# bharatlytics/faceRecognition_InfrenceEngine

Measured on AMD Instinct MI355X. Metric: faces/sec end-to-end @1080p, higher is better.
Workload: dtype f16

## Files before the change

### facerecognition_infrenceengine_amd/csrc/common.h

```cpp
#pragma once
#include <hip/hip_runtime.h>
#include <atomic>
#include <cstdarg>
#include <cstdint>
#include <cstdio>
#include <type_traits>
#include "../../include/frhip.h"

#define FR_WAVE 64

void fr_set_error(const char* fmt, ...);

#define FR_REQUIRE(cond, ...)                      \
    do {                                           \
        if (!(cond)) {                             \
            fr_set_error(__VA_ARGS__);             \
            return FR_E_INVALID;                   \
        }                                          \
    } while (0)

#define FR_CHECK_LAUNCH(name)                                                     \
    do {                                                                          \
        hipError_t e_ = hipGetLastError();                                        \
        if (e_ != hipSuccess) {                                                   \
// ... 22 lines not shown
typedef _Float16 half2v __attribute__((ext_vector_type(2)));
typedef float float4v __attribute__((ext_vector_type(4)));
typedef float float16v __attribute__((ext_vector_type(16)));
typedef int int2v __attribute__((ext_vector_type(2)));
typedef int int4v __attribute__((ext_vector_type(4)));
typedef int int8v __attribute__((ext_vector_type(8)));
typedef __attribute__((address_space(3))) void* lds_ptr_t;
typedef unsigned long long u64_unaligned __attribute__((aligned(1)));

template <int N, int I = 0, class F>
__device__ __forceinline__ void static_for(F&& f) {
    if constexpr (I < N) {
        f(std::integral_constant<int, I>{});
        static_for<N, I + 1>(f);
    }
}

#define FR_PIN() __builtin_amdgcn_sched_barrier(0)

__device__ __forceinline__ float wave_sum(float v) {
#pragma unroll
    for (int o = 32; o > 0; o >>= 1) v += __shfl_xor(v, o, 64);
    return v;
}

__device__ __forceinline__ __amdgpu_buffer_rsrc_t buffer_rsrc(const void* p, unsigned bytes) {
    return __builtin_amdgcn_make_buffer_rsrc((void*)p, 0, bytes, 0x00020000);
}

__device__ __forceinline__ float4v mfma16(const int4v& a, const int4v& b, float4v c) {
    return __builtin_amdgcn_mfma_f32_16x16x32_f16(__builtin_bit_cast(half8, a), __builtin_bit_cast(half8, b), c, 0, 0, 0);
}

__device__ __forceinline__ int pack_fp8x4(float a, float b, float c, float d) {
    a = __builtin_amdgcn_fmed3f(a, -448.f, 448.f); b = __builtin_amdgcn_fmed3f(b, -448.f, 448.f);
    c = __builtin_amdgcn_fmed3f(c, -448.f, 448.f); d = __builtin_amdgcn_fmed3f(d, -448.f, 448.f);
    int v = 0;
    v = __builtin_amdgcn_cvt_pk_fp8_f32(a, b, v, false);
    v = __builtin_amdgcn_cvt_pk_fp8_f32(c, d, v, true);
    return v;
}

__device__ __forceinline__ bool slot_valid(const int32_t* seg_counts, int seg_len, int q) {
    const int seg = q / seg_len;
    return q - seg * seg_len < seg_counts[seg];
}
```

### facerecognition_infrenceengine_amd/csrc/conv_stage28.hip

```cpp
#include "common.h"
#include <type_traits>

namespace {

constexpr int S28_W = 28, S28_TH = 14, S28_C = 128;
constexpr int S28_HROWS = 16 * 32;
constexpr int S28_PLANE = S28_HROWS * 128;
constexpr int S28_SLOT = 128 * 64;
constexpr int S28_STEPS = 36;
constexpr int S28_PRM = 10 * 128 * 4;
constexpr int S28_RING = 2 * S28_PLANE, S28_PRMO = S28_RING + 3 * S28_SLOT;
constexpr int S28_LDS = S28_PRMO + S28_PRM;
constexpr int S28_PX = S28_TH * S28_W;
constexpr int S28_IMG = 784 * S28_C * 2;

struct Stage28P {
    half_t* x; half_t* mid; const half_t* w; const float* prm;
    int B, nconv;
    unsigned xbytes, wbytes;
};

}

__global__ __launch_bounds__(512, 2) void conv_stage28_kernel(Stage28P p) {
#if defined(__HIP_DEVICE_COMPILE__)
    extern __shared__ __attribute__((aligned(16))) char lds[];
    char* ring = lds + S28_RING;
    const float* lprm = reinterpret_cast<const float*>(lds + S28_PRMO);
    const int tid = threadIdx.x;
    const int wave = __builtin_amdgcn_readfirstlane(tid >> 6);
    const int wn = wave & 1, wp = wave >> 1;
    const int n = blockIdx.x;

    __amdgpu_buffer_rsrc_t wrs = buffer_rsrc(p.w, p.wbytes);
    __amdgpu_buffer_rsrc_t xrs = buffer_rsrc(p.x, p.xbytes);
    __amdgpu_buffer_rsrc_t mrs = buffer_rsrc(p.mid, p.xbytes);
    __amdgpu_buffer_rsrc_t prs = buffer_rsrc(p.prm, (unsigned)p.nconv * S28_PRM);

    unsigned wsrc = 0, wwrap = S28_STEPS * S28_SLOT, wback = 0;
    auto issue_w = [&](int slot, int ln) {
        __builtin_amdgcn_raw_ptr_buffer_load_lds(wrs, (lds_ptr_t)(ring + slot * S28_SLOT + wave * 1024), 16,
                                                 wsrc < p.wbytes ? (unsigned)(wave * 1024 + ln * 16) : 0x80000000u, wsrc, 0, 0);
        wsrc += S28_SLOT;
        if (wsrc == wwrap) wsrc = wback;
    };
    auto halo_lane = [&](int ln) -> unsigned {
        const int lrow = ln >> 3, ch = ln & 7, q = wave & 3;
        const unsigned out = (unsigned)((q == 0) & (lrow == 0)) | (unsigned)((q == 3) & (lrow >= 5));
        return ((unsigned)((lrow - 1) * 256 + ((ch ^ ((lrow + 4 * ((wave >> 2) & 1)) & 7)) << 4)) & (out - 1u)) | (out << 31);
    };
    auto issue_halo = [&](__amdgpu_buffer_rsrc_t rs, int plane, int i, int y0, unsigned lt, bool src_ok) {
        int n_ = n;
        asm volatile("" : "+s"(n_));
        const int hy = 2 * i + (wave >> 2), iy = y0 - 1 + hy;
        const bool ok = src_ok && (unsigned)iy < 28u;
        const unsigned so = (unsigned)(((n_ * 28 + iy) * 28 + (wave & 3) * 8) * 256 + plane * 128);
        __builtin_amdgcn_raw_ptr_buffer_load_lds(rs, (lds_ptr_t)(lds + plane * S28_PLANE + (hy * 4 + (wave & 3)) * 1024), 16,
                                                 ok ? lt + so : 0x80000000u, 0, 0, 16);
    };
    auto issue_prm = [&](int conv, int ln) {
        if (wave < 5)
            __builtin_amdgcn_raw_ptr_buffer_load_lds(prs, (lds_ptr_t)(lds + S28_PRMO + wave * 1024), 16, (unsigned)(wave * 1024 + ln * 16), conv * S28_PRM, 0, 0);
    };

    {
        const int ln = tid & 63;
        issue_w(0, ln);
        issue_w(1, ln);
        issue_w(2, ln);
        issue_prm(0, ln);
        const unsigned lt = halo_lane(ln);
        for (int i = 0; i < 16; ++i) issue_halo(xrs, i >> 3, i & 7, 0, lt, true);
    }

    float4v acc[6][4], accx;
    int4v a0[4], a1[4], bt[3], bx;
    int boff[7];

    auto run = [&](auto role_tag) {
    constexpr int ROLE = decltype(role_tag)::value;
#pragma unroll 1
    for (int pass = 0; pass < 2 * p.nconv; ++pass) {
        const int conv = pass >> 1, hf = pass & 1, y0 = hf * S28_TH;
        int lane = tid & 63;
        asm volatile("" : "+v"(lane));
        const int fr = lane & 15, fq = lane >> 4;
        const bool second = conv & 1;
        __amdgpu_buffer_rsrc_t srs = second ? mrs : xrs;
        __amdgpu_buffer_rsrc_t nxr = hf == 0 ? srs : (second ? xrs : mrs);
        const int nxy0 = hf == 0 ? S28_TH : 0;
        const bool nx_any = hf == 0 || conv + 1 < p.nconv;
        auto nx_ok = [&](int i) { return nx_any && (hf == 0 || !(i == 7 && (wave >> 2) == 1)); };
        half_t* dst = second ? p.x : p.mid;
        const unsigned tile0 = (unsigned)((n * 28 + y0) * 28);
        int a_own = fr * 64 + ((fq ^ (((fr >> 3) & 1) << 1)) << 4);
        asm volatile("" : "+v"(a_own));
        int hb[6];
#pragma unroll
        for (int j = 0; j < 6; ++j) {
            const int px = (wp * 6 + j) * 16 + fr;
            const int oy = px / S28_W, ox = px - oy * S28_W;
            hb[j] = (oy + 1) * 32 + ox + 1;
            asm volatile("" : "+v"(hb[j]));
        }
        auto set_tap_one = [&](int j, int dy, int dx, int plane) {
            int l_ = lane;
            asm volatile("" : "+v"(l_));
            const int h = (j < 6 ? hb[j < 6 ? j : 0] : ((l_ & 15) < 8 ? 14 * 32 + 21 + (l_ & 15) : 33)) + dy * 32 + dx;
            boff[j] = plane * S28_PLANE + h * 128 + (((l_ >> 4) ^ ((((h >> 3) & 4) + h) & 7)) << 4);
        };
        auto rd_a = [&](int slot, int i) {
            return *reinterpret_cast<const int4v*>(ring + slot * S28_SLOT + (wn * 4096 + ((i + wp) & 3) * 1024) + a_own);
        };
        auto rd_b = [&](int gg, int j) { return *reinterpret_cast<const int4v*>(lds + (gg ? (boff[j] ^ 64) : boff[j])); };
        auto co_of = [&](int i) { return wn * 64 + ((i + wp) & 3) * 16 + fq * 4; };

        if (hf == 0) {
            if (pass == 0) asm volatile("s_waitcnt vmcnt(16)" ::: "memory");
            else if (wave >> 2) asm volatile("s_waitcnt vmcnt(2)" ::: "memory");
            else asm volatile("s_waitcnt vmcnt(0)" ::: "memory");
            __builtin_amdgcn_s_barrier();
        }
        auto cls_off = [&](int px) {
            const int oy = px / S28_W, ox = px - oy * S28_W, ho = y0 + oy;
            return ((ho == 0 ? 0 : (ho == 27 ? 2 : 1)) * 3 + (ox == 0 ? 0 : (ox == 27 ? 2 : 1))) * S28_C;
        };
#pragma unroll
        for (int j = 0; j < 6; ++j) {
            const int cj = cls_off((wp * 6 + j) * 16 + fr);
#pragma unroll
            for (int i = 0; i < 4; ++i) acc[j][i] = *reinterpret_cast<const float4v*>(lprm + cj + co_of(i));
        }
        accx = *reinterpret_cast<const float4v*>(lprm + cls_off(fr < 8 ? 384 + fr : 0) + co_of(0));
        auto co8 = [&](int ip) { return wn * 64 + ((ip + (fq & 1) + wp) & 3) * 16 + (fq >> 1) * 8; };
        if (second) {
            int4v r[6][2];
#pragma unroll
            for (int j = 0; j < 6; ++j)
#pragma unroll
                for (int ip = 0; ip < 2; ++ip)
                    r[j][ip] = __builtin_bit_cast(int4v, __builtin_amdgcn_raw_buffer_load_b128(
                        xrs, (tile0 + (unsigned)((wp * 6 + j) * 16 + fr)) * 256u + (unsigned)co8(2 * ip) * 2u, 0, 16));
#pragma unroll
            for (int j = 0; j < 6; ++j)
#pragma unroll
                for (int ip = 0; ip < 2; ++ip) {
                    const auto s0 = __builtin_amdgcn_permlane16_swap((unsigned)r[j][ip][0], (unsigned)r[j][ip][2], false, false);
                    const auto s1 = __builtin_amdgcn_permlane16_swap((unsigned)r[j][ip][1], (unsigned)r[j][ip][3], false, false);
                    const half4 ha = __builtin_bit_cast(half4, int2v{(int)s0[0], (int)s1[0]});
                    const half4 hb_ = __builtin_bit_cast(half4, int2v{(int)s0[1], (int)s1[1]});
#pragma unroll
                    for (int e = 0; e < 4; ++e) { acc[j][2 * ip][e] += (float)ha[e]; acc[j][2 * ip + 1][e] += (float)hb_[e]; }
                }
            const int2v rx = __builtin_bit_cast(int2v, __builtin_amdgcn_raw_buffer_load_b64(
                xrs, fr < 8 ? (tile0 + (unsigned)(384 + fr)) * 256u + (unsigned)co_of(0) * 2u : 0x80000000u, 0, 16));
            const half4 hx = __builtin_bit_cast(half4, rx);
#pragma unroll
            for (int e = 0; e < 4; ++e) accx[e] += (float)hx[e];
        }
        asm volatile("s_waitcnt vmcnt(0)" ::: "memory");
        __builtin_amdgcn_s_barrier();
        wwrap = (unsigned)(conv + 1) * (S28_STEPS * S28_SLOT);
        wback = hf == 0 ? (unsigned)conv * (S28_STEPS * S28_SLOT) : wwrap;

#pragma unroll
        for (int j = 0; j < 7; ++j) set_tap_one(j, -1, -1, 0);
#pragma unroll
        for (int i = 0; i < 4; ++i) a0[i] = rd_a(0, i);
#pragma unroll
        for (int j = 0; j < 3; ++j) bt[j] = rd_b(0, j);
        bx = rd_b(0, 6);

        auto step = [&](int4v (&ac)[4], int4v (&an)[4], int k, int dyn, int dxn, int pln, auto pf_tag) {
            constexpr bool PF = decltype(pf_tag)::value;
            const int gg = k & 1, ngg = (k + 1) & 1, nslot = (k + 1) % 3;
            auto dma = [&]() {
                if constexpr (PF) {
                    if (k < 4) {
                        int l_ = lane;
                        asm volatile("" : "+v"(l_));
                        const unsigned ltp = halo_lane(l_);
                        issue_halo(nxr, 0, 2 * k, nxy0, ltp, nx_ok(2 * k));
                        issue_halo(nxr, 0, 2 * k + 1, nxy0, ltp, nx_ok(2 * k + 1));
                    }
                }
                issue_w(k % 3, lane);
            };
            if constexpr (ROLE == 0) { dma(); FR_PIN(); }
            accx = mfma16(ac[0], bx, accx);
            FR_PIN();
#pragma unroll
            for (int j = 0; j < 6; ++j) {
#pragma unroll
                for (int i = 0; i < 4; ++i) acc[j][i] = mfma16(ac[i], bt[j % 3], acc[j][i]);
                if (j == 0) { an[0] = rd_a(nslot, 0); an[1] = rd_a(nslot, 1); }
                if (j == 1) { an[2] = rd_a(nslot, 2); an[3] = rd_a(nslot, 3); }
                if (j < 3) {
                    bt[j] = rd_b(gg, j + 3);
                } else {
                    if (gg == 1) { set_tap_one(j - 3, dyn, dxn, pln); set_tap_one(j, dyn, dxn, pln); }
                    bt[j - 3] = rd_b(ngg, j - 3);
                    if (j == 5) {
                        if (gg == 1) set_tap_one(6, dyn, dxn, pln);
                        bx = rd_b(ngg, 6);
                    }
                }
                FR_PIN();
                if constexpr (ROLE == 1) { if (j == 3) { dma(); FR_PIN(); } }
            }
        };
        auto row = [&](int it, int plane, auto pf_tag) {
            constexpr bool PF = decltype(pf_tag)::value;
#pragma unroll
            for (int k = 0; k < 6; ++k) {
                if (PF && k >= 1 && k <= 4) asm volatile("s_waitcnt vmcnt(3) lgkmcnt(1)" ::: "memory");
                else asm volatile("s_waitcnt vmcnt(1) lgkmcnt(1)" ::: "memory");
                __builtin_amdgcn_s_barrier();
                FR_PIN();
                const int tt = k >> 1;
                const bool last = tt == 2 && it == 2;
                const int dyn = last ? -1 : (tt < 2 ? it - 1 : it), dxn = tt < 2 ? tt : -1;
                const int pln = last ? (plane ^ 1) & 1 : plane;
                if ((k & 1) == 0) step(a0, a1, k, dyn, dxn, pln, pf_tag);
                else step(a1, a0, k, dyn, dxn, pln, pf_tag);
            }
        };
#pragma unroll 1
        for (int it = 0; it < 3; ++it) row(it, 0, std::false_type{});
        row(0, 1, std::true_type{});
#pragma unroll 1
        for (int it = 1; it < 3; ++it) row(it, 1, std::false_type{});

        asm volatile("s_waitcnt lgkmcnt(0)" ::: "memory");
        __builtin_amdgcn_s_barrier();
        int le = lane;
        asm volatile("" : "+v"(le));
        const unsigned lt = halo_lane(le);
        for (int i = 0; i < 8; ++i) issue_halo(nxr, 1, i, nxy0, lt, nx_ok(i));
        FR_PIN();
        const int fre = le & 15, fqe = le >> 4;
        auto coe = [&](int i) { return wn * 64 + ((i + wp) & 3) * 16 + fqe * 4; };
        float4v sv[4];
#pragma unroll
        for (int i = 0; i < 4; ++i) sv[i] = *reinterpret_cast<const float4v*>(lprm + 9 * S28_C + coe(i));
        auto act = [&](float4v v, int i) {
            if (!second) {
#pragma unroll
                for (int e = 0; e < 4; ++e) v[e] = v[e] > 0.f ? v[e] : v[e] * sv[i][e];
            }
            return __builtin_bit_cast(int2v, half4{(half_t)v[0], (half_t)v[1], (half_t)v[2], (half_t)v[3]});
        };
        auto co8e = [&](int ip) { return wn * 64 + ((ip + (fqe & 1) + wp) & 3) * 16 + (fqe >> 1) * 8; };
#pragma unroll
        for (int j = 0; j < 6; ++j)
#pragma unroll
            for (int ip = 0; ip < 2; ++ip) {
                const int2v pa = act(acc[j][2 * ip], 2 * ip), pb = act(acc[j][2 * ip + 1], 2 * ip + 1);
                const auto s0 = __builtin_amdgcn_permlane16_swap((unsigned)pa[0], (unsigned)pb[0], false, false);
                const auto s1 = __builtin_amdgcn_permlane16_swap((unsigned)pa[1], (unsigned)pb[1], false, false);
                *reinterpret_cast<int4v*>(dst + (size_t)(tile0 + (wp * 6 + j) * 16 + fre) * S28_C + co8e(2 * ip)) =
                    int4v{(int)s0[0], (int)s1[0], (int)s0[1], (int)s1[1]};
            }
        if (fre < 8)
            *reinterpret_cast<int2v*>(dst + (size_t)(tile0 + 384 + fre) * S28_C + coe(0)) = act(accx, 0);
        if (hf == 1) {
            asm volatile("s_waitcnt vmcnt(0)" ::: "memory");
            __builtin_amdgcn_s_barrier();
            if (conv + 1 < p.nconv) {
                issue_prm(conv + 1, lane);
                if (wave >> 2) {
                    issue_halo(nxr, 0, 7, 0, lt, true);
                    issue_halo(nxr, 1, 7, 0, lt, true);
                }
            }
        }
    }
    };
    if ((wp >> 1) == 0) run(std::integral_constant<int, 0>{}); else run(std::integral_constant<int, 1>{});
    asm volatile("s_waitcnt vmcnt(0) lgkmcnt(0)" ::: "memory");
#endif
}

extern "C" size_t fr_conv_stage28_weight_bytes(int nconv) { return nconv > 0 ? (size_t)nconv * S28_STEPS * S28_SLOT : 0; }

__global__ void stage28_pack_weights(const half_t* __restrict__ w, half_t* __restrict__ out) {
    const int e = blockIdx.x * blockDim.x + threadIdx.x;
    if (e >= S28_STEPS * 512) return;
    const int q = e / 512, r = e - q * 512, row = r >> 2, cp = r & 3;
    const int chunk = cp ^ (((row >> 3) & 1) << 1);
    const int plane = q / 18, k = q - plane * 18, tap = k >> 1, gg = k & 1;
    const int4v v = *reinterpret_cast<const int4v*>(w + (size_t)row * 1152 + tap * 128 + plane * 64 + gg * 32 + chunk * 8);
    *reinterpret_cast<int4v*>(out + (size_t)q * 4096 + row * 32 + cp * 8) = v;
}

extern "C" int fr_conv_stage28_pack(const void* w, void* out, fr_stream_t stream) {
    FR_REQUIRE(w && out, "fr_conv_stage28_pack: null pointer");
    stage28_pack_weights<<<fr_cdiv(S28_STEPS * 512, 256), 256, 0, fr_stream(stream)>>>((const half_t*)w, (half_t*)out);
// ... 24 lines not shown
```

### facerecognition_infrenceengine_amd/csrc/conv_walk64.hip

```cpp
#include "common.h"
#include <type_traits>

namespace {

constexpr int K64_RW = 28, K64_RH = 14, K64_C = 64;
constexpr int K64_PX = K64_RW * K64_RH;
constexpr int K64_HALO = 512 * 128;
constexpr int K64_SLOT = 64 * 128;
constexpr int K64_RING = 2 * K64_HALO, K64_PRMO = K64_RING + 3 * K64_SLOT;
constexpr int K64_PRM = 10 * 64 * 4;
constexpr int K64_LDS = K64_PRMO + K64_PRM;

struct Walk64P {
    const half_t* x; const half_t* w; half_t* y;
    const float* bias; const float* slope; const half_t* res;
    int B, HW, Cout, bias_mode;
    int nsplit;
    unsigned xbytes, ybytes, wbytes;
};

}

__global__ __launch_bounds__(512, 2) void conv_walk64_kernel(Walk64P p) {
#if defined(__HIP_DEVICE_COMPILE__)
    extern __shared__ __attribute__((aligned(16))) char lds[];
    char* ring = lds + K64_RING;
    float* lprm = reinterpret_cast<float*>(lds + K64_PRMO);
    const int tid = threadIdx.x;
    const int wave = __builtin_amdgcn_readfirstlane(tid >> 6);
    const int ncg = p.Cout >> 6;
    const int cg = blockIdx.x % ncg, part = (blockIdx.x / ncg) % p.nsplit, n = blockIdx.x / (ncg * p.nsplit);
    const int HW = p.HW, nbx = HW / K64_RW;
    const int reg0 = part * (nbx * (HW / K64_RH) / p.nsplit), nreg = reg0 + nbx * (HW / K64_RH) / p.nsplit;

    __amdgpu_buffer_rsrc_t wrs = buffer_rsrc(p.w, p.wbytes);
    __amdgpu_buffer_rsrc_t xrs = buffer_rsrc(p.x, p.xbytes);

    const unsigned wbase = (unsigned)cg * (9 * K64_SLOT);
    unsigned wq = 0;
    auto issue_w = [&](int slot, int ln) {
        __builtin_amdgcn_raw_ptr_buffer_load_lds(wrs, (lds_ptr_t)(ring + slot * K64_SLOT + wave * 1024), 16,
                                                 (unsigned)(wave * 1024 + ln * 16), wbase + wq * K64_SLOT, 0, 0);
        wq = wq == 8 ? 0 : wq + 1;
    };
    auto halo_lane = [&](int ln, bool left_edge, bool right_edge) -> unsigned {
        const int lrow = ln >> 3, ch = ln & 7, q = wave & 3;
        const unsigned out = (unsigned)((q == 0) & (lrow == 0) & left_edge) | (unsigned)((q == 3) & (lrow == 5) & right_edge) |
                             (unsigned)((q == 3) & (lrow >= 6));
        return ((unsigned)((lrow - 1) * 128 + ((ch ^ ((lrow + 4 * ((wave >> 2) & 1)) & 7)) << 4)) & (out - 1u)) | (out << 31);
    };
    auto issue_halo = [&](int buf, int i, int reg, int ln) {
        int n_ = n;
        asm volatile("" : "+s"(n_));
        const int by = reg / nbx, bx_ = reg - by * nbx;
        const int y0 = by * K64_RH, x0 = bx_ * K64_RW;
        const unsigned lt = halo_lane(ln, x0 == 0, x0 + K64_RW == HW);
        const int hy = 2 * i + (wave >> 2), iy = y0 - 1 + hy;
        const bool ok = reg < nreg && (unsigned)iy < (unsigned)HW;
        const unsigned so = (unsigned)(((n_ * HW + iy) * HW + x0 + (wave & 3) * 8) * 128);
        __builtin_amdgcn_raw_ptr_buffer_load_lds(xrs, (lds_ptr_t)(lds + buf * K64_HALO + (hy * 4 + (wave & 3)) * 1024), 16,
                                                 ok ? lt + so : 0x80000000u, 0, 0, 0);
    };

    {
        const int ln = tid & 63;
        issue_w(0, ln);
        issue_w(1, ln);
        issue_w(2, ln);
        for (int i = 0; i < 8; ++i) issue_halo(reg0 & 1, i, reg0, ln);
        for (int e = tid; e < 640; e += 512) {
            const int r = e >> 6, c = e & 63;
            float v;
            if (r < 9) v = p.bias ? p.bias[(p.bias_mode == 1 ? r * p.Cout : 0) + cg * 64 + c] : 0.f;
            else v = p.slope ? p.slope[cg * 64 + c] : 1.f;
            lprm[e] = v;
        }
    }

    float4v acc[3][4], accx;
    int4v a0[2][4], a1[2][4], b[3][2], bx[2];
    int boff[4];

    auto run = [&](auto role_tag) {
    constexpr int ROLE = decltype(role_tag)::value;
#pragma unroll 1
    for (int reg = reg0; reg < nreg; ++reg) {
        const int cur = reg & 1;
        int lane = tid & 63;
        asm volatile("" : "+v"(lane));
        const int fr = lane & 15, fq = lane >> 4;
        const int by = reg / nbx, bx_ = reg - by * nbx;
        const int y0 = by * K64_RH, x0 = bx_ * K64_RW;
        auto gpix = [&](int px) {
            const int oy = px / K64_RW, ox = px - oy * K64_RW;
            return (unsigned)((n * HW + y0 + oy) * HW + x0 + ox);
        };
        auto cls_off = [&](int px) {
            const int oy = px / K64_RW, ox = px - oy * K64_RW, ho = y0 + oy, wo = x0 + ox;
            return ((ho == 0 ? 0 : (ho == HW - 1 ? 2 : 1)) * 3 + (wo == 0 ? 0 : (wo == HW - 1 ? 2 : 1))) * 64;
        };
        auto ct = [&](int f) { return (f + wave) & 3; };
        auto co8 = [&](int ip) { return ct(2 * ip + (fq & 1)) * 16 + (fq >> 1) * 8; };
        int a_own = fr * 128 + ((fq ^ (fr & 7)) << 4);
        asm volatile("" : "+v"(a_own));
        int hb[3];
#pragma unroll
        for (int t = 0; t < 3; ++t) {
            const int px = (wave * 3 + t) * 16 + fr;
            const int oy = px / K64_RW, ox = px - oy * K64_RW;
            hb[t] = (oy + 1) * 32 + ox + 1;
            asm volatile("" : "+v"(hb[t]));
        }
        auto set_tap_one = [&](int t, int dy, int dx) {
            int l_ = lane;
            asm volatile("" : "+v"(l_));
            const int h = (t < 3 ? hb[t < 3 ? t : 0] : ((l_ & 15) < 8 ? 14 * 32 + 21 + (l_ & 15) : 33)) + dy * 32 + dx;
            boff[t] = cur * K64_HALO + h * 128 + (((l_ >> 4) ^ ((((h >> 3) & 4) + h) & 7)) << 4);
        };
        auto rd_a = [&](int slot, int kh, int i) { return *reinterpret_cast<const int4v*>(ring + slot * K64_SLOT + ct(i) * 2048 + (kh ? (a_own ^ 64) : a_own)); };
        auto rd_b = [&](int kh, int t) { return *reinterpret_cast<const int4v*>(lds + (kh ? (boff[t] ^ 64) : boff[t])); };

        asm volatile("s_waitcnt lgkmcnt(0)" ::: "memory");
        if (reg == reg0) __builtin_amdgcn_s_barrier();
#pragma unroll
        for (int t = 0; t < 3; ++t) {
            const int cj = cls_off((wave * 3 + t) * 16 + fr);
#pragma unroll
            for (int i = 0; i < 4; ++i) acc[t][i] = *reinterpret_cast<const float4v*>(lprm + cj + ct(i) * 16 + fq * 4);
        }
        accx = *reinterpret_cast<const float4v*>(lprm + cls_off(fr < 8 ? 384 + fr : 0) + (wave & 3) * 16 + fq * 4);
        if (p.res) {
            __amdgpu_buffer_rsrc_t rrs = buffer_rsrc(p.res, p.ybytes);
            int4v r[3][2];
#pragma unroll
            for (int t = 0; t < 3; ++t)
#pragma unroll
                for (int ip = 0; ip < 2; ++ip)
                    r[t][ip] = __builtin_bit_cast(int4v, __builtin_amdgcn_raw_buffer_load_b128(
                        rrs, (gpix((wave * 3 + t) * 16 + fr) * (unsigned)p.Cout + (unsigned)(cg * 64 + co8(ip))) * 2u, 0, 16));
            const int2v rx = __builtin_bit_cast(int2v, __builtin_amdgcn_raw_buffer_load_b64(
                rrs, fr < 8 ? (gpix(384 + fr) * (unsigned)p.Cout + (unsigned)(cg * 64 + (wave & 3) * 16 + fq * 4)) * 2u : 0x80000000u, 0, 16));
#pragma unroll
            for (int t = 0; t < 3; ++t)
#pragma unroll
                for (int ip = 0; ip < 2; ++ip) {
                    const auto s0 = __builtin_amdgcn_permlane16_swap((unsigned)r[t][ip][0], (unsigned)r[t][ip][2], false, false);
                    const auto s1 = __builtin_amdgcn_permlane16_swap((unsigned)r[t][ip][1], (unsigned)r[t][ip][3], false, false);
                    const half4 ha = __builtin_bit_cast(half4, int2v{(int)s0[0], (int)s1[0]});
                    const half4 hb_ = __builtin_bit_cast(half4, int2v{(int)s0[1], (int)s1[1]});
#pragma unroll
                    for (int e = 0; e < 4; ++e) { acc[t][2 * ip][e] += (float)ha[e]; acc[t][2 * ip + 1][e] += (float)hb_[e]; }
                }
            const half4 hx = __builtin_bit_cast(half4, rx);
#pragma unroll
            for (int e = 0; e < 4; ++e) accx[e] += (float)hx[e];
        }
        asm volatile("s_waitcnt vmcnt(0)" ::: "memory");
        __builtin_amdgcn_s_barrier();

#pragma unroll
        for (int t = 0; t < 4; ++t) set_tap_one(t, -1, -1);
#pragma unroll
        for (int kh = 0; kh < 2; ++kh) {
#pragma unroll
            for (int i = 0; i < 4; ++i) a0[kh][i] = rd_a(0, kh, i);
#pragma unroll
            for (int t = 0; t < 3; ++t) b[t][kh] = rd_b(kh, t);
            bx[kh] = rd_b(kh, 3);
        }

        auto step = [&](int4v (&ac)[2][4], int4v (&an)[2][4], int s) {
            const int nslot = (s + 1) % 3;
            const int tn = s + 1 < 9 ? s + 1 : 0;
            const int dyn = tn / 3 - 1, dxn = tn % 3 - 1;
            auto dma = [&]() {
                if (s < 8) issue_halo(cur ^ 1, s, reg + 1, lane);
                issue_w(s % 3, lane);
            };
            if constexpr (ROLE == 0) { dma(); FR_PIN(); }
#pragma unroll
            for (int kh = 0; kh < 2; ++kh) {
                accx = mfma16(ac[kh][0], bx[kh], accx);
                FR_PIN();
#pragma unroll
                for (int t = 0; t < 3; ++t) {
#pragma unroll
                    for (int i = 0; i < 4; ++i) acc[t][i] = mfma16(ac[kh][i], b[t][kh], acc[t][i]);
                    if (kh == 0) { an[0][t] = rd_a(nslot, 0, t); if (t == 2) an[0][3] = rd_a(nslot, 0, 3); }
                    else { an[1][t] = rd_a(nslot, 1, t); if (t == 2) an[1][3] = rd_a(nslot, 1, 3); }
                    if (kh == 0) set_tap_one(t, dyn, dxn);
                    b[t][kh] = rd_b(kh, t);
                    if (t == 2) {
                        if (kh == 0) set_tap_one(3, dyn, dxn);
                        bx[kh] = rd_b(kh, 3);
                    }
                    FR_PIN();
                }
                if constexpr (ROLE == 1) { if (kh == 0) { dma(); FR_PIN(); } }
            }
        };
#pragma unroll
        for (int s = 0; s < 9; ++s) {
            asm volatile("s_waitcnt vmcnt(2) lgkmcnt(1)" ::: "memory");
            __builtin_amdgcn_s_barrier();
            FR_PIN();
            if ((s & 1) == 0) step(a0, a1, s); else step(a1, a0, s);
        }

        asm volatile("s_waitcnt lgkmcnt(0)" ::: "memory");
        int le = lane;
        asm volatile("" : "+v"(le));
        const int fre = le & 15, fqe = le >> 4;
        float4v sv[4];
#pragma unroll
        for (int i = 0; i < 4; ++i) sv[i] = *reinterpret_cast<const float4v*>(lprm + 9 * 64 + ct(i) * 16 + fqe * 4);
        auto act = [&](float4v v, const float4v& s_) {
#pragma unroll
            for (int e = 0; e < 4; ++e) v[e] = v[e] > 0.f ? v[e] : v[e] * s_[e];
            return __builtin_bit_cast(int2v, half4{(half_t)v[0], (half_t)v[1], (half_t)v[2], (half_t)v[3]});
        };
        half_t* yo = p.y + cg * 64;
#pragma unroll
        for (int t = 0; t < 3; ++t) {
            const size_t gp = (size_t)gpix((wave * 3 + t) * 16 + fre) * p.Cout;
#pragma unroll
            for (int ip = 0; ip < 2; ++ip) {
                const int2v pa = act(acc[t][2 * ip], sv[2 * ip]), pb = act(acc[t][2 * ip + 1], sv[2 * ip + 1]);
                const auto s0 = __builtin_amdgcn_permlane16_swap((unsigned)pa[0], (unsigned)pb[0], false, false);
                const auto s1 = __builtin_amdgcn_permlane16_swap((unsigned)pa[1], (unsigned)pb[1], false, false);
                *reinterpret_cast<int4v*>(yo + gp + ct(2 * ip + (fqe & 1)) * 16 + (fqe >> 1) * 8) = int4v{(int)s0[0], (int)s1[0], (int)s0[1], (int)s1[1]};
            }
        }
        if (wave < 4 && fre < 8)
            *reinterpret_cast<int2v*>(yo + (size_t)gpix(384 + fre) * p.Cout + wave * 16 + fqe * 4) = act(accx, sv[0]);
    }
    };
    if ((wave >> 2) == 0) run(std::integral_constant<int, 0>{}); else run(std::integral_constant<int, 1>{});
    asm volatile("s_waitcnt vmcnt(0) lgkmcnt(0)" ::: "memory");
#endif
}

extern "C" size_t fr_conv_walk64_weight_bytes(int Cout) { return Cout > 0 ? (size_t)(Cout / 64) * 9 * K64_SLOT : 0; }

__global__ void walk64_pack_weights(const half_t* __restrict__ w, half_t* __restrict__ out, int ncg) {
    const int e = blockIdx.x * blockDim.x + threadIdx.x;
    if (e >= ncg * 9 * 512) return;
    const int q_ = e / 512, r = e - q_ * 512, row = r >> 3, cp = r & 7;
    const int cgi = q_ / 9, tap = q_ - cgi * 9;
    const int chunk = cp ^ (row & 7);
    const int4v v = *reinterpret_cast<const int4v*>(w + (size_t)(cgi * 64 + row) * 576 + tap * 64 + chunk * 8);
    *reinterpret_cast<int4v*>(out + (size_t)q_ * 4096 + row * 64 + cp * 8) = v;
}

extern "C" int fr_conv_walk64_pack(const void* w, void* out, int Cout, fr_stream_t stream) {
    FR_REQUIRE(w && out && Cout > 0 && Cout % 64 == 0, "fr_conv_walk64_pack: bad argument (Cout %d)", Cout);
    const int ncg = Cout / 64;
    walk64_pack_weights<<<fr_cdiv((int64_t)ncg * 9 * 512, 256), 256, 0, fr_stream(stream)>>>((const half_t*)w, (half_t*)out, ncg);
    FR_CHECK_LAUNCH("walk64_pack_weights");
    return FR_OK;
}

extern "C" int fr_conv_walk64_f16(const void* x, const void* wstream, void* y, const float* bias, int bias_mode, const float* slope,
                                  const void* residual, int B, int HW, int Cout, fr_stream_t stream) {
    FR_REQUIRE(x && wstream && y && B > 0, "fr_conv_walk64_f16: bad argument");
    FR_REQUIRE(x != y, "fr_conv_walk64_f16: y must not alias x");
    FR_REQUIRE(HW > 0 && HW % 28 == 0 && Cout > 0 && Cout % 64 == 0, "fr_conv_walk64_f16: image side %d must be a multiple of 28, Cout %d of 64", HW, Cout);
    FR_REQUIRE(bias_mode == 0 || bias_mode == 1, "fr_conv_walk64_f16: bad bias_mode");
// ... 22 lines not shown
```

Baseline: 26990.

## Precompute B-operand tap addresses and use max-based PReLU with buffer stores

```diff
diff --git a/facerecognition_infrenceengine_amd/csrc/common.h b/facerecognition_infrenceengine_amd/csrc/common.h
--- a/facerecognition_infrenceengine_amd/csrc/common.h
+++ b/facerecognition_infrenceengine_amd/csrc/common.h
@@ -78,6 +78,16 @@
     return __builtin_amdgcn_mfma_f32_16x16x32_f16(__builtin_bit_cast(half8, a), __builtin_bit_cast(half8, b), c, 0, 0, 0);
 }
 
+__device__ __forceinline__ float prelu_max(float v, float m) {
+    float r;
+    asm("v_max_f32 %0, %1, %2" : "=v"(r) : "v"(v), "v"(m));
+    return r;
+}
+__device__ __forceinline__ bool slope_unit(const float4v& s) {
+    const int4v u = __builtin_bit_cast(int4v, s);
+    return (unsigned)u[0] <= 0x3f800000u && (unsigned)u[1] <= 0x3f800000u && (unsigned)u[2] <= 0x3f800000u && (unsigned)u[3] <= 0x3f800000u;
+}
+
 __device__ __forceinline__ int pack_fp8x4(float a, float b, float c, float d) {
     a = __builtin_amdgcn_fmed3f(a, -448.f, 448.f); b = __builtin_amdgcn_fmed3f(b, -448.f, 448.f);
     c = __builtin_amdgcn_fmed3f(c, -448.f, 448.f); d = __builtin_amdgcn_fmed3f(d, -448.f, 448.f);
diff --git a/facerecognition_infrenceengine_amd/csrc/conv_stage28.hip b/facerecognition_infrenceengine_amd/csrc/conv_stage28.hip
--- a/facerecognition_infrenceengine_amd/csrc/conv_stage28.hip
+++ b/facerecognition_infrenceengine_amd/csrc/conv_stage28.hip
@@ -10,8 +10,9 @@
 constexpr int S28_STEPS = 36;
 constexpr int S28_PRM = 10 * 128 * 4;
 constexpr int S28_RING = 2 * S28_PLANE, S28_PRMO = S28_RING + 3 * S28_SLOT;
-constexpr int S28_LDS = S28_PRMO + S28_PRM;
 constexpr int S28_PX = S28_TH * S28_W;
+constexpr int S28_TBLO = S28_PRMO + S28_PRM;
+constexpr int S28_LDS = S28_TBLO + S28_PX * 4;
 constexpr int S28_IMG = 784 * S28_C * 2;
 
 struct Stage28P {
@@ -31,6 +32,7 @@
     const int wave = __builtin_amdgcn_readfirstlane(tid >> 6);
     const int wn = wave & 1, wp = wave >> 1;
     const int n = blockIdx.x;
+    if ((unsigned)(size_t)(lds_ptr_t)lds != 0u) return;
 
     __amdgpu_buffer_rsrc_t wrs = buffer_rsrc(p.w, p.wbytes);
     __amdgpu_buffer_rsrc_t xrs = buffer_rsrc(p.x, p.xbytes);
@@ -71,6 +73,11 @@
         issue_prm(0, ln);
         const unsigned lt = halo_lane(ln);
         for (int i = 0; i < 16; ++i) issue_halo(xrs, i >> 3, i & 7, 0, lt, true);
+        if (tid < S28_PX) {
+            const int oy = tid / S28_W, ox = tid - oy * S28_W, cc = ox == 0 ? 0 : (ox == 27 ? 2 : 1), key = 4 * (oy & 1) + ox;
+            reinterpret_cast<int*>(lds + S28_TBLO)[tid] = ((oy * 32 + ox) * 128) | ((key & 7) << 4) | (((key + 1) & 7) << 21) | (((key + 2) & 7) << 28) |
+                                                          ((oy == 0 ? 0 : 1) * 3 + cc) | (((oy == 13 ? 2 : 1) * 3 + cc) << 17);
+        }
     }
 
     float4v acc[6][4], accx;
@@ -91,56 +98,54 @@
         const int nxy0 = hf == 0 ? S28_TH : 0;
         const bool nx_any = hf == 0 || conv + 1 < p.nconv;
         auto nx_ok = [&](int i) { return nx_any && (hf == 0 || !(i == 7 && (wave >> 2) == 1)); };
-        half_t* dst = second ? p.x : p.mid;
         const unsigned tile0 = (unsigned)((n * 28 + y0) * 28);
         int a_own = fr * 64 + ((fq ^ (((fr >> 3) & 1) << 1)) << 4);
         asm volatile("" : "+v"(a_own));
-        int hb[6];
-#pragma unroll
-        for (int j = 0; j < 6; ++j) {
-            const int px = (wp * 6 + j) * 16 + fr;
-            const int oy = px / S28_W, ox = px - oy * S28_W;
-            hb[j] = (oy + 1) * 32 + ox + 1;
-            asm volatile("" : "+v"(hb[j]));
-        }
-        auto set_tap_one = [&](int j, int dy, int dx, int plane) {
-            int l_ = lane;
-            asm volatile("" : "+v"(l_));
-            const int h = (j < 6 ? hb[j < 6 ? j : 0] : ((l_ & 15) < 8 ? 14 * 32 + 21 + (l_ & 15) : 33)) + dy * 32 + dx;
-            boff[j] = plane * S28_PLANE + h * 128 + (((l_ >> 4) ^ ((((h >> 3) & 4) + h) & 7)) << 4);
-        };
+        int frag[7];
+        constexpr int FRAG_ROW = 64 | (64 << 17) | (64 << 24);
+        auto set_tap_one = [&](int j, int tx) {
+            boff[j] = tx == 0 ? (frag[j] & 0x1ffff) : ((frag[j] & 0x1ff80) | ((frag[j] >> (tx == 1 ? 17 : 24)) & 0x7f));
+        };
+        auto next_row = [&](int j, bool last) {
+            const int fx = last ? S28_PLANE : FRAG_ROW, fa = last ? -2 * 4096 : 4096;
+            frag[j] = (frag[j] ^ fx) + fa;
+        };
+        typedef const __attribute__((address_space(3))) int4v* lds_frag_t;
         auto rd_a = [&](int slot, int i) {
             return *reinterpret_cast<const int4v*>(ring + slot * S28_SLOT + (wn * 4096 + ((i + wp) & 3) * 1024) + a_own);
         };
-        auto rd_b = [&](int gg, int j) { return *reinterpret_cast<const int4v*>(lds + (gg ? (boff[j] ^ 64) : boff[j])); };
+        auto rd_b = [&](int gg, int j, int tx) { return *(lds_frag_t)(unsigned)((gg ? (boff[j] ^ 64) : boff[j]) + tx * 128); };
         auto co_of = [&](int i) { return wn * 64 + ((i + wp) & 3) * 16 + fq * 4; };
 
         if (hf == 0) {
-            if (pass == 0) asm volatile("s_waitcnt vmcnt(16)" ::: "memory");
+            if (pass == 0) asm volatile("s_waitcnt vmcnt(16) lgkmcnt(0)" ::: "memory");
             else if (wave >> 2) asm volatile("s_waitcnt vmcnt(2)" ::: "memory");
             else asm volatile("s_waitcnt vmcnt(0)" ::: "memory");
             __builtin_amdgcn_s_barrier();
         }
-        auto cls_off = [&](int px) {
-            const int oy = px / S28_W, ox = px - oy * S28_W, ho = y0 + oy;
-            return ((ho == 0 ? 0 : (ho == 27 ? 2 : 1)) * 3 + (ox == 0 ? 0 : (ox == 27 ? 2 : 1))) * S28_C;
-        };
-#pragma unroll
-        for (int j = 0; j < 6; ++j) {
-            const int cj = cls_off((wp * 6 + j) * 16 + fr);
-#pragma unroll
-            for (int i = 0; i < 4; ++i) acc[j][i] = *reinterpret_cast<const float4v*>(lprm + cj + co_of(i));
-        }
-        accx = *reinterpret_cast<const float4v*>(lprm + cls_off(fr < 8 ? 384 + fr : 0) + co_of(0));
+        const int* ltbl = reinterpret_cast<const int*>(lds + S28_TBLO);
+        const int csh = 17 * hf;
+        const int fq3 = (fq << 4) | (fq << 21) | (fq << 28);
+#pragma unroll
+        for (int j = 0; j < 7; ++j) {
+            const int e_ = ltbl[j < 6 ? (wp * 6 + j) * 16 + fr : (fr < 8 ? 384 + fr : 0)];
+            frag[j] = (e_ & ~(15 | (15 << 17))) ^ fq3;
+            asm volatile("" : "+v"(frag[j]));
+            const int cj = ((e_ >> csh) & 15) * S28_C;
+            if (j < 6) {
+#pragma unroll
+                for (int i = 0; i < 4; ++i) acc[j][i] = *reinterpret_cast<const float4v*>(lprm + cj + co_of(i));
+            } else accx = *reinterpret_cast<const float4v*>(lprm + cj + co_of(0));
+        }
         auto co8 = [&](int ip) { return wn * 64 + ((ip + (fq & 1) + wp) & 3) * 16 + (fq >> 1) * 8; };
         if (second) {
             int4v r[6][2];
+            const unsigned pv = (unsigned)((wp * 6 * 16 + fr) * 256 + co8(0) * 2);
 #pragma unroll
             for (int j = 0; j < 6; ++j)
 #pragma unroll
                 for (int ip = 0; ip < 2; ++ip)
-                    r[j][ip] = __builtin_bit_cast(int4v, __builtin_amdgcn_raw_buffer_load_b128(
-                        xrs, (tile0 + (unsigned)((wp * 6 + j) * 16 + fr)) * 256u + (unsigned)co8(2 * ip) * 2u, 0, 16));
+                    r[j][ip] = __builtin_bit_cast(int4v, __builtin_amdgcn_raw_buffer_load_b128(xrs, ip ? pv ^ 64u : pv, tile0 * 256u + (unsigned)(j * 4096), 16));
 #pragma unroll
             for (int j = 0; j < 6; ++j)
 #pragma unroll
@@ -164,16 +169,17 @@
         wback = hf == 0 ? (unsigned)conv * (S28_STEPS * S28_SLOT) : wwrap;
 
 #pragma unroll
-        for (int j = 0; j < 7; ++j) set_tap_one(j, -1, -1, 0);
+        for (int j = 0; j < 7; ++j) set_tap_one(j, 0);
 #pragma unroll
         for (int i = 0; i < 4; ++i) a0[i] = rd_a(0, i);
 #pragma unroll
-        for (int j = 0; j < 3; ++j) bt[j] = rd_b(0, j);
-        bx = rd_b(0, 6);
-
-        auto step = [&](int4v (&ac)[4], int4v (&an)[4], int k, int dyn, int dxn, int pln, auto pf_tag) {
+        for (int j = 0; j < 3; ++j) bt[j] = rd_b(0, j, 0);
+        bx = rd_b(0, 6, 0);
+
+        auto step = [&](int4v (&ac)[4], int4v (&an)[4], int k, bool last, auto pf_tag) {
             constexpr bool PF = decltype(pf_tag)::value;
             const int gg = k & 1, ngg = (k + 1) & 1, nslot = (k + 1) % 3;
+            const int tx = k >> 1, ntx = gg == 1 ? (tx + 1) % 3 : tx;
             auto dma = [&]() {
                 if constexpr (PF) {
                     if (k < 4) {
@@ -195,14 +201,18 @@
                 for (int i = 0; i < 4; ++i) acc[j][i] = mfma16(ac[i], bt[j % 3], acc[j][i]);
                 if (j == 0) { an[0] = rd_a(nslot, 0); an[1] = rd_a(nslot, 1); }
                 if (j == 1) { an[2] = rd_a(nslot, 2); an[3] = rd_a(nslot, 3); }
+                auto next_tap = [&](int jj) {
+                    if (k == 5) next_row(jj, last);
+                    set_tap_one(jj, ntx);
+                };
                 if (j < 3) {
-                    bt[j] = rd_b(gg, j + 3);
+                    bt[j] = rd_b(gg, j + 3, tx);
                 } else {
-                    if (gg == 1) { set_tap_one(j - 3, dyn, dxn, pln); set_tap_one(j, dyn, dxn, pln); }
-                    bt[j - 3] = rd_b(ngg, j - 3);
+                    if (gg == 1) { next_tap(j - 3); next_tap(j); }
+                    bt[j - 3] = rd_b(ngg, j - 3, ntx);
                     if (j == 5) {
-                        if (gg == 1) set_tap_one(6, dyn, dxn, pln);
-                        bx = rd_b(ngg, 6);
+                        if (gg == 1) next_tap(6);
+                        bx = rd_b(ngg, 6, ntx);
                     }
                 }
                 FR_PIN();
@@ -217,12 +227,9 @@
                 else asm volatile("s_waitcnt vmcnt(1) lgkmcnt(1)" ::: "memory");
                 __builtin_amdgcn_s_barrier();
                 FR_PIN();
-                const int tt = k >> 1;
-                const bool last = tt == 2 && it == 2;
-                const int dyn = last ? -1 : (tt < 2 ? it - 1 : it), dxn = tt < 2 ? tt : -1;
-                const int pln = last ? (plane ^ 1) & 1 : plane;
-                if ((k & 1) == 0) step(a0, a1, k, dyn, dxn, pln, pf_tag);
-                else step(a1, a0, k, dyn, dxn, pln, pf_tag);
+                const bool last = it == 2;
+                if ((k & 1) == 0) step(a0, a1, k, last, pf_tag);
+                else step(a1, a0, k, last, pf_tag);
             }
         };
 #pragma unroll 1
@@ -243,26 +250,36 @@
         float4v sv[4];
 #pragma unroll
         for (int i = 0; i < 4; ++i) sv[i] = *reinterpret_cast<const float4v*>(lprm + 9 * S28_C + coe(i));
-        auto act = [&](float4v v, int i) {
-            if (!second) {
-#pragma unroll
-                for (int e = 0; e < 4; ++e) v[e] = v[e] > 0.f ? v[e] : v[e] * sv[i][e];
-            }
-            return __builtin_bit_cast(int2v, half4{(half_t)v[0], (half_t)v[1], (half_t)v[2], (half_t)v[3]});
-        };
-        auto co8e = [&](int ip) { return wn * 64 + ((ip + (fqe & 1) + wp) & 3) * 16 + (fqe >> 1) * 8; };
-#pragma unroll
-        for (int j = 0; j < 6; ++j)
-#pragma unroll
-            for (int ip = 0; ip < 2; ++ip) {
-                const int2v pa = act(acc[j][2 * ip], 2 * ip), pb = act(acc[j][2 * ip + 1], 2 * ip + 1);
-                const auto s0 = __builtin_amdgcn_permlane16_swap((unsigned)pa[0], (unsigned)pb[0], false, false);
-                const auto s1 = __builtin_amdgcn_permlane16_swap((unsigned)pa[1], (unsigned)pb[1], false, false);
-                *reinterpret_cast<int4v*>(dst + (size_t)(tile0 + (wp * 6 + j) * 16 + fre) * S28_C + co8e(2 * ip)) =
-                    int4v{(int)s0[0], (int)s1[0], (int)s0[1], (int)s1[1]};
-            }
-        if (fre < 8)
-            *reinterpret_cast<int2v*>(dst + (size_t)(tile0 + 384 + fre) * S28_C + coe(0)) = act(accx, 0);
+        const bool unit = __builtin_amdgcn_ballot_w64(slope_unit(sv[0]) && slope_unit(sv[1]) && slope_unit(sv[2]) && slope_unit(sv[3])) == ~0ull;
+        __amdgpu_buffer_rsrc_t drs = second ? xrs : mrs;
+        const unsigned pve = (unsigned)((wp * 6 * 16 + fre) * 256 + (wn * 64 + (((fqe & 1) + wp) & 3) * 16 + (fqe >> 1) * 8) * 2);
+        auto store = [&](auto mode_tag) {
+            constexpr int MODE = decltype(mode_tag)::value;
+            auto act = [&](float4v v, int i) {
+#pragma unroll
+                for (int e = 0; e < 4; ++e) {
+                    if constexpr (MODE == 1) v[e] = prelu_max(v[e], v[e] * sv[i][e]);
+                    if constexpr (MODE == 2) v[e] = v[e] > 0.f ? v[e] : v[e] * sv[i][e];
+                }
+                return __builtin_bit_cast(int2v, half4{(half_t)v[0], (half_t)v[1], (half_t)v[2], (half_t)v[3]});
+            };
+#pragma unroll
+            for (int j = 0; j < 6; ++j)
+#pragma unroll
+                for (int ip = 0; ip < 2; ++ip) {
+                    const int2v pa = act(acc[j][2 * ip], 2 * ip), pb = act(acc[j][2 * ip + 1], 2 * ip + 1);
+                    const auto s0 = __builtin_amdgcn_permlane16_swap((unsigned)pa[0], (unsigned)pb[0], false, false);
+                    const auto s1 = __builtin_amdgcn_permlane16_swap((unsigned)pa[1], (unsigned)pb[1], false, false);
+                    __builtin_amdgcn_raw_buffer_store_b128(__builtin_bit_cast(__attribute__((ext_vector_type(4))) unsigned, int4v{(int)s0[0], (int)s1[0], (int)s0[1], (int)s1[1]}),
+                                                           drs, ip ? pve ^ 64u : pve, tile0 * 256u + (unsigned)(j * 4096), 0);
+                }
+            if (fre < 8)
+                __builtin_amdgcn_raw_buffer_store_b64(__builtin_bit_cast(__attribute__((ext_vector_type(2))) unsigned, act(accx, 0)), drs,
+                                                      (unsigned)((384 + fre) * 256 + coe(0) * 2), tile0 * 256u, 0);
+        };
+        if (second) store(std::integral_constant<int, 0>{});
+        else if (unit) store(std::integral_constant<int, 1>{});
+        else store(std::integral_constant<int, 2>{});
         if (hf == 1) {
             asm volatile("s_waitcnt vmcnt(0)" ::: "memory");
             __builtin_amdgcn_s_barrier();
diff --git a/facerecognition_infrenceengine_amd/csrc/conv_walk64.hip b/facerecognition_infrenceengine_amd/csrc/conv_walk64.hip
--- a/facerecognition_infrenceengine_amd/csrc/conv_walk64.hip
+++ b/facerecognition_infrenceengine_amd/csrc/conv_walk64.hip
@@ -8,7 +8,7 @@
 constexpr int K64_HALO = 512 * 128;
 constexpr int K64_SLOT = 64 * 128;
 constexpr int K64_RING = 2 * K64_HALO, K64_PRMO = K64_RING + 3 * K64_SLOT;
-constexpr int K64_PRM = 10 * 64 * 4;
+constexpr int K64_PRM = 12 * 64 * 4;
 constexpr int K64_LDS = K64_PRMO + K64_PRM;
 
 struct Walk64P {
@@ -68,67 +68,97 @@
         issue_w(1, ln);
         issue_w(2, ln);
         for (int i = 0; i < 8; ++i) issue_halo(reg0 & 1, i, reg0, ln);
-        for (int e = tid; e < 640; e += 512) {
-            const int r = e >> 6, c = e & 63;
-            float v;
-            if (r < 9) v = p.bias ? p.bias[(p.bias_mode == 1 ? r * p.Cout : 0) + cg * 64 + c] : 0.f;
-            else v = p.slope ? p.slope[cg * 64 + c] : 1.f;
+        for (int e = tid; e < 768; e += 512) {
+            const int r = e >> 6, c = e & 63, f_r = r >> 2, f_c = r & 3;
+            float v = 0.f;
+            if (r == 11) v = p.slope ? p.slope[cg * 64 + c] : 1.f;
+            else if (f_c < 3) {
+                const int cl = (f_r == 0 ? 1 : f_r == 1 ? 0 : 2) * 3 + (f_c == 0 ? 1 : f_c == 1 ? 0 : 2);
+                v = p.bias ? p.bias[(p.bias_mode == 1 ? cl * p.Cout : 0) + cg * 64 + c] : 0.f;
+            }
             lprm[e] = v;
         }
     }
 
     float4v acc[3][4], accx;
     int4v a0[2][4], a1[2][4], b[3][2], bx[2];
-    int boff[4];
 
     auto run = [&](auto role_tag) {
     constexpr int ROLE = decltype(role_tag)::value;
+    const int lane = tid & 63, fr = lane & 15, fq = lane >> 4, q = wave & 3;
+    auto ct = [&](int f) { return (f + wave) & 3; };
+    auto co8 = [&](int ip) { return ct(2 * ip + (fq & 1)) * 16 + (fq >> 1) * 8; };
+    int baddr[4][6];
+    int yoff[3][2], yoffx;
+    int cls[4];
+#pragma unroll
+    for (int t = 0; t < 4; ++t) {
+        const int px = t < 3 ? (wave * 3 + t) * 16 + fr : (fr < 8 ? 384 + fr : 0);
+        const int oy = px / K64_RW, ox = px - oy * K64_RW;
+        const int key0 = 4 * (oy & 1) + ox;
+#pragma unroll
+        for (int j = 0; j < 6; ++j) {
+            const int c = j < 3 ? j : j + 1;
+            baddr[t][j] = (reg0 & 1) * K64_HALO + (oy * 32 + ox) * 128 + ((fq ^ ((key0 + c) & 7)) << 4);
+        }
+        cls[t] = ((oy == 0) << 10) | ((oy == K64_RH - 1) << 11) | ((ox == 0) << 8) | ((ox == K64_RW - 1) << 9);
+        const int po = (oy * p.HW + ox) * p.Cout;
+        if (t < 3) { yoff[t][0] = (po + co8(0)) * 2; yoff[t][1] = (po + co8(1)) * 2; }
+        else yoffx = (po + q * 16 + fq * 4) * 2;
+    }
+    int aaddr[2][4];
+#pragma unroll
+    for (int kh = 0; kh < 2; ++kh)
+#pragma unroll
+        for (int i = 0; i < 4; ++i) aaddr[kh][i] = K64_RING + ct(i) * 2048 + ((fr * 128 + ((fq ^ (fr & 7)) << 4)) ^ (kh * 64));
+    const int prm_lane = K64_PRMO + fq * 16;
+    const unsigned w_lane = (unsigned)(wave * 1024 + lane * 16);
+    auto rd_a = [&](int slot, int kh, int i) { return *reinterpret_cast<const int4v*>(lds + aaddr[kh][i] + slot * K64_SLOT); };
+    auto rd_b = [&](int kh, int t, int tap) {
+        const int ty = tap / 3, tx = tap % 3, c = (4 * (ty & 1) + tx + 4 * kh) & 7;
+        return *reinterpret_cast<const int4v*>(lds + baddr[t][c < 3 ? c : c - 1] + (ty * 32 + tx) * 128);
+    };
+    auto issue_wl = [&](int slot) {
+        __builtin_amdgcn_raw_ptr_buffer_load_lds(wrs, (lds_ptr_t)(ring + slot * K64_SLOT + wave * 1024), 16, w_lane, wbase + wq * K64_SLOT, 0, 0);
+        wq = wq == 8 ? 0 : wq + 1;
+    };
+
+    asm volatile("s_waitcnt lgkmcnt(0)" ::: "memory");
+    __builtin_amdgcn_s_barrier();
+    bool mono;
+    {
+        bool m = true;
+#pragma unroll
+        for (int i = 0; i < 4; ++i) m = m && slope_unit(*reinterpret_cast<const float4v*>(lds + prm_lane + 11 * 256 + ct(i) * 64));
+        mono = __builtin_amdgcn_ballot_w64(m) == ~0ull;
+    }
+
+    const int Cout2 = p.Cout * 2;
+    int by = reg0 / nbx, bxr = reg0 - by * nbx;
 #pragma unroll 1
     for (int reg = reg0; reg < nreg; ++reg) {
         const int cur = reg & 1;
-        int lane = tid & 63;
-        asm volatile("" : "+v"(lane));
-        const int fr = lane & 15, fq = lane >> 4;
-        const int by = reg / nbx, bx_ = reg - by * nbx;
-        const int y0 = by * K64_RH, x0 = bx_ * K64_RW;
-        auto gpix = [&](int px) {
-            const int oy = px / K64_RW, ox = px - oy * K64_RW;
-            return (unsigned)((n * HW + y0 + oy) * HW + x0 + ox);
+        const int y0 = by * K64_RH, x0 = bxr * K64_RW;
+        const int edges = ((y0 == 0) << 10) | ((y0 + K64_RH == HW) << 11) | ((x0 == 0) << 8) | ((x0 + K64_RW == HW) << 9);
+        const unsigned ybase = (unsigned)((n * HW + y0) * HW + x0) * (unsigned)Cout2 + (unsigned)(cg * 128);
+        if (++bxr == nbx) { bxr = 0; ++by; }
+        const int y0n = by * K64_RH, x0n = bxr * K64_RW;
+        const unsigned ltn = halo_lane(lane, x0n == 0, x0n + K64_RW == HW);
+        const int iyn = y0n - 1 + ROLE;
+        const unsigned son = (unsigned)(((n * HW + iyn) * HW + x0n + q * 8) * 128);
+        auto issue_halo_next = [&](int i) {
+            const bool ok = reg + 1 < nreg && (unsigned)(iyn + 2 * i) < (unsigned)HW;
+            __builtin_amdgcn_raw_ptr_buffer_load_lds(xrs, (lds_ptr_t)(lds + (cur ^ 1) * K64_HALO + ((2 * i + ROLE) * 4 + q) * 1024), 16,
+                                                     ok ? ltn + son + (unsigned)(2 * i * HW * 128) : 0x80000000u, 0, 0, 0);
         };
-        auto cls_off = [&](int px) {
-            const int oy = px / K64_RW, ox = px - oy * K64_RW, ho = y0 + oy, wo = x0 + ox;
-            return ((ho == 0 ? 0 : (ho == HW - 1 ? 2 : 1)) * 3 + (wo == 0 ? 0 : (wo == HW - 1 ? 2 : 1))) * 64;
-        };
-        auto ct = [&](int f) { return (f + wave) & 3; };
-        auto co8 = [&](int ip) { return ct(2 * ip + (fq & 1)) * 16 + (fq >> 1) * 8; };
-        int a_own = fr * 128 + ((fq ^ (fr & 7)) << 4);
-        asm volatile("" : "+v"(a_own));
-        int hb[3];
+
 #pragma unroll
         for (int t = 0; t < 3; ++t) {
-            const int px = (wave * 3 + t) * 16 + fr;
-            const int oy = px / K64_RW, ox = px - oy * K64_RW;
-            hb[t] = (oy + 1) * 32 + ox + 1;
-            asm volatile("" : "+v"(hb[t]));
-        }
-        auto set_tap_one = [&](int t, int dy, int dx) {
-            int l_ = lane;
-            asm volatile("" : "+v"(l_));
-            const int h = (t < 3 ? hb[t < 3 ? t : 0] : ((l_ & 15) < 8 ? 14 * 32 + 21 + (l_ & 15) : 33)) + dy * 32 + dx;
-            boff[t] = cur * K64_HALO + h * 128 + (((l_ >> 4) ^ ((((h >> 3) & 4) + h) & 7)) << 4);
-        };
-        auto rd_a = [&](int slot, int kh, int i) { return *reinterpret_cast<const int4v*>(ring + slot * K64_SLOT + ct(i) * 2048 + (kh ? (a_own ^ 64) : a_own)); };
-        auto rd_b = [&](int kh, int t) { return *reinterpret_cast<const int4v*>(lds + (kh ? (boff[t] ^ 64) : boff[t])); };
-
-        asm volatile("s_waitcnt lgkmcnt(0)" ::: "memory");
-        if (reg == reg0) __builtin_amdgcn_s_barrier();
-#pragma unroll
-        for (int t = 0; t < 3; ++t) {
-            const int cj = cls_off((wave * 3 + t) * 16 + fr);
-#pragma unroll
-            for (int i = 0; i < 4; ++i) acc[t][i] = *reinterpret_cast<const float4v*>(lprm + cj + ct(i) * 16 + fq * 4);
-        }
-        accx = *reinterpret_cast<const float4v*>(lprm + cls_off(fr < 8 ? 384 + fr : 0) + (wave & 3) * 16 + fq * 4);
+            const int cj = (cls[t] & edges) | prm_lane;
+#pragma unroll
+            for (int i = 0; i < 4; ++i) acc[t][i] = *reinterpret_cast<const float4v*>(lds + cj + ct(i) * 64);
+        }
+        accx = *reinterpret_cast<const float4v*>(lds + ((cls[3] & edges) | prm_lane) + q * 64);
         if (p.res) {
             __amdgpu_buffer_rsrc_t rrs = buffer_rsrc(p.res, p.ybytes);
             int4v r[3][2];
@@ -136,10 +166,8 @@
             for (int t = 0; t < 3; ++t)
 #pragma unroll
                 for (int ip = 0; ip < 2; ++ip)
-                    r[t][ip] = __builtin_bit_cast(int4v, __builtin_amdgcn_raw_buffer_load_b128(
-                        rrs, (gpix((wave * 3 + t) * 16 + fr) * (unsigned)p.Cout + (unsigned)(cg * 64 + co8(ip))) * 2u, 0, 16));
-            const int2v rx = __builtin_bit_cast(int2v, __builtin_amdgcn_raw_buffer_load_b64(
-                rrs, fr < 8 ? (gpix(384 + fr) * (unsigned)p.Cout + (unsigned)(cg * 64 + (wave & 3) * 16 + fq * 4)) * 2u : 0x80000000u, 0, 16));
+                    r[t][ip] = __builtin_bit_cast(int4v, __builtin_amdgcn_raw_buffer_load_b128(rrs, yoff[t][ip], ybase, 16));
+            const int2v rx = __builtin_bit_cast(int2v, __builtin_amdgcn_raw_buffer_load_b64(rrs, yoffx, ybase, 16));
 #pragma unroll
             for (int t = 0; t < 3; ++t)
 #pragma unroll
@@ -159,23 +187,20 @@
         __builtin_amdgcn_s_barrier();
 
 #pragma unroll
-        for (int t = 0; t < 4; ++t) set_tap_one(t, -1, -1);
-#pragma unroll
         for (int kh = 0; kh < 2; ++kh) {
 #pragma unroll
             for (int i = 0; i < 4; ++i) a0[kh][i] = rd_a(0, kh, i);
 #pragma unroll
-            for (int t = 0; t < 3; ++t) b[t][kh] = rd_b(kh, t);
-            bx[kh] = rd_b(kh, 3);
+            for (int t = 0; t < 3; ++t) b[t][kh] = rd_b(kh, t, 0);
+            bx[kh] = rd_b(kh, 3, 0);
         }
 
         auto step = [&](int4v (&ac)[2][4], int4v (&an)[2][4], int s) {
             const int nslot = (s + 1) % 3;
             const int tn = s + 1 < 9 ? s + 1 : 0;
-            const int dyn = tn / 3 - 1, dxn = tn % 3 - 1;
             auto dma = [&]() {
-                if (s < 8) issue_halo(cur ^ 1, s, reg + 1, lane);
-                issue_w(s % 3, lane);
+                if (s < 8) issue_halo_next(s);
+                issue_wl(s % 3);
             };
             if constexpr (ROLE == 0) { dma(); FR_PIN(); }
 #pragma unroll
@@ -188,12 +213,8 @@
                     for (int i = 0; i < 4; ++i) acc[t][i] = mfma16(ac[kh][i], b[t][kh], acc[t][i]);
                     if (kh == 0) { an[0][t] = rd_a(nslot, 0, t); if (t == 2) an[0][3] = rd_a(nslot, 0, 3); }
                     else { an[1][t] = rd_a(nslot, 1, t); if (t == 2) an[1][3] = rd_a(nslot, 1, 3); }
-                    if (kh == 0) set_tap_one(t, dyn, dxn);
-                    b[t][kh] = rd_b(kh, t);
-                    if (t == 2) {
-                        if (kh == 0) set_tap_one(3, dyn, dxn);
-                        bx[kh] = rd_b(kh, 3);
-                    }
+                    b[t][kh] = rd_b(kh, t, tn);
+                    if (t == 2) bx[kh] = rd_b(kh, 3, tn);
                     FR_PIN();
                 }
                 if constexpr (ROLE == 1) { if (kh == 0) { dma(); FR_PIN(); } }
@@ -208,31 +229,38 @@
         }
 
         asm volatile("s_waitcnt lgkmcnt(0)" ::: "memory");
-        int le = lane;
-        asm volatile("" : "+v"(le));
-        const int fre = le & 15, fqe = le >> 4;
-        float4v sv[4];
-#pragma unroll
-        for (int i = 0; i < 4; ++i) sv[i] = *reinterpret_cast<const float4v*>(lprm + 9 * 64 + ct(i) * 16 + fqe * 4);
-        auto act = [&](float4v v, const float4v& s_) {
-#pragma unroll
-            for (int e = 0; e < 4; ++e) v[e] = v[e] > 0.f ? v[e] : v[e] * s_[e];
-            return __builtin_bit_cast(int2v, half4{(half_t)v[0], (half_t)v[1], (half_t)v[2], (half_t)v[3]});
+        __amdgpu_buffer_rsrc_t yrs = buffer_rsrc(p.y, p.ybytes);
+        auto store = [&](auto mono_tag) {
+            constexpr bool MONO = decltype(mono_tag)::value;
+            float4v sv[4];
+#pragma unroll
+            for (int i = 0; i < 4; ++i) sv[i] = *reinterpret_cast<const float4v*>(lds + prm_lane + 11 * 256 + ct(i) * 64);
+            auto act = [&](float4v v, const float4v& s_) {
+#pragma unroll
+                for (int e = 0; e < 4; ++e) {
+                    if constexpr (MONO) v[e] = prelu_max(v[e], v[e] * s_[e]);
+                    else v[e] = v[e] > 0.f ? v[e] : v[e] * s_[e];
+                }
+                return __builtin_bit_cast(int2v, half4{(half_t)v[0], (half_t)v[1], (half_t)v[2], (half_t)v[3]});
+            };
+#pragma unroll
+            for (int t = 0; t < 3; ++t)
+#pragma unroll
+                for (int ip = 0; ip < 2; ++ip) {
+                    const int2v pa = act(acc[t][2 * ip], sv[2 * ip]), pb = act(acc[t][2 * ip + 1], sv[2 * ip + 1]);
+                    const auto s0 = __builtin_amdgcn_permlane16_swap((unsigned)pa[0], (unsigned)pb[0], false, false);
+                    const auto s1 = __builtin_amdgcn_permlane16_swap((unsigned)pa[1], (unsigned)pb[1], false, false);
+                    __builtin_amdgcn_raw_buffer_store_b128(__builtin_bit_cast(__attribute__((ext_vector_type(4))) unsigned, int4v{(int)s0[0], (int)s1[0], (int)s0[1], (int)s1[1]}),
+                                                           yrs, yoff[t][ip], ybase, 0);
+                }
+            if (wave < 4 && fr < 8)
+                __builtin_amdgcn_raw_buffer_store_b64(__builtin_bit_cast(__attribute__((ext_vector_type(2))) unsigned, act(accx, sv[0])), yrs, yoffx, ybase, 0);
         };
-        half_t* yo = p.y + cg * 64;
-#pragma unroll
-        for (int t = 0; t < 3; ++t) {
-            const size_t gp = (size_t)gpix((wave * 3 + t) * 16 + fre) * p.Cout;
-#pragma unroll
-            for (int ip = 0; ip < 2; ++ip) {
-                const int2v pa = act(acc[t][2 * ip], sv[2 * ip]), pb = act(acc[t][2 * ip + 1], sv[2 * ip + 1]);
-                const auto s0 = __builtin_amdgcn_permlane16_swap((unsigned)pa[0], (unsigned)pb[0], false, false);
-                const auto s1 = __builtin_amdgcn_permlane16_swap((unsigned)pa[1], (unsigned)pb[1], false, false);
-                *reinterpret_cast<int4v*>(yo + gp + ct(2 * ip + (fqe & 1)) * 16 + (fqe >> 1) * 8) = int4v{(int)s0[0], (int)s1[0], (int)s0[1], (int)s1[1]};
-            }
-        }
-        if (wave < 4 && fre < 8)
-            *reinterpret_cast<int2v*>(yo + (size_t)gpix(384 + fre) * p.Cout + wave * 16 + fqe * 4) = act(accx, sv[0]);
+        if (mono) store(std::true_type{}); else store(std::false_type{});
+#pragma unroll
+        for (int t = 0; t < 4; ++t)
+#pragma unroll
+            for (int j = 0; j < 6; ++j) baddr[t][j] ^= K64_HALO;
     }
     };
     if ((wave >> 2) == 0) run(std::integral_constant<int, 0>{}); else run(std::integral_constant<int, 1>{});
```

Measured after the change: 27440 (median of 5 runs). 1.02x the previous value.
